# NVIDIA-Genomics-Research/DL4VC

Hardware: AMD Instinct MI355X
Metric: candidate-variants/sec (DAN fwd, 64 reads x 201 bp) (higher is better)
Workload: dtype f32

## Files before the change

### dl4vc_amd/capi.py

```python
from __future__ import annotations

import ctypes as C
import os
from typing import Dict, Optional

import numpy as np

from .config import DanConfig

_HERE = os.path.dirname(os.path.abspath(__file__))
LIB_PATH = os.path.join(_HERE, "csrc", "libdl4vc_dan.so")
ABI_VERSION = 6

SYMBOLS = ("dan_abi_version", "dan_source_hash", "dan_create", "dan_set_tensor", "dan_finalize", "dan_destroy", "dan_last_error",
           "dan_forward", "dan_forward_aux", "dan_forward_device", "dan_forward_async", "dan_wait", "dan_set_tap", "dan_read_buffer", "dan_query",
           "dan_profile_enable", "dan_kernel_stats")


class DanCConfig(C.Structure):
    _fields_ = [("reads", C.c_int32), ("length", C.c_int32), ("layers", C.c_int32), ("c_init", C.c_int32),
                ("c_final", C.c_int32), ("dil_mid", C.c_int32), ("dil_final", C.c_int32),
                ("pool_layers_mask", C.c_uint32), ("residual_start", C.c_int32), ("use_bn", C.c_int32),
                ("use_q", C.c_int32), ("use_strand", C.c_int32), ("use_mask", C.c_int32), ("bottleneck", C.c_int32),
                ("fc_sizes", C.c_int32 * 2), ("precision", C.c_int32), ("device_id", C.c_int32),
                ("max_batch", C.c_int32), ("chunk_sites", C.c_int32), ("conv_algo", C.c_int32), ("skip_empty_rows", C.c_int32),
                ("bf16_form", C.c_int32)]


_lib = None

# ... 16 lines not shown
    lib.dan_destroy.argtypes = [vp]
    lib.dan_destroy.restype = None
    lib.dan_last_error.argtypes = [vp]
    lib.dan_last_error.restype = C.c_char_p
    planes = [vp] * 6
    lib.dan_forward.argtypes = [vp] + planes + [C.c_int64] + [vp] * 4
    lib.dan_forward_aux.argtypes = [vp] + planes + [C.c_int64] + [vp] * 5
    lib.dan_forward_device.argtypes = [vp] + planes + [C.c_int64] + [vp] * 5 + [vp]
    lib.dan_forward_async.argtypes = [vp] + planes + [C.c_int64] + [vp] * 5 + [C.POINTER(C.c_int64)]
    lib.dan_wait.argtypes = [vp, C.c_int64]
    lib.dan_set_tap.argtypes = [vp, C.c_int32]
    lib.dan_read_buffer.argtypes = [vp, C.c_char_p, f32p, C.c_int64]
    lib.dan_read_buffer.restype = C.c_int64
    lib.dan_query.argtypes = [vp, C.c_char_p]
    lib.dan_query.restype = C.c_int64
    lib.dan_profile_enable.argtypes = [vp, C.c_int32]
    lib.dan_kernel_stats.argtypes = [vp, C.c_char_p, C.POINTER(C.c_int64), C.POINTER(C.c_double)]
    if lib.dan_abi_version() != ABI_VERSION:
        raise RuntimeError("libdl4vc_dan ABI %d != binding %d" % (lib.dan_abi_version(), ABI_VERSION))
    if path is None:
        _lib = lib
    return lib


def source_hash() -> str:
    return load_library().dan_source_hash().decode()


HASHED_SOURCES = ("dan_*.hip", "dan_*.h", "dan_capi.cpp", "dan_train_capi.cpp")

# ... 118 lines not shown
        ticket, out = token
        self._check(self.lib.dan_wait(self._h, ticket), "dan_wait")
        if "aux" in out:
            a = out.pop("aux")
            out.update(af=a[:, 0:1].copy(), cov=a[:, 1:2].copy(), vb=a[:, 2:12].copy(), vr=a[:, 12:22].copy())
        return out

    def forward_device(self, ptrs, n_sites: int, out_ptrs, stream: int = 0) -> None:
        v = lambda x: C.c_void_p(int(x)) if x else None
        rc = self.lib.dan_forward_device(self._h, *[v(x) for x in ptrs], int(n_sites), *[v(x) for x in out_ptrs], v(stream))
        self._check(rc, "dan_forward_device")

    def set_tap(self, layer: int) -> None:
        self._check(self.lib.dan_set_tap(self._h, layer), "dan_set_tap")

    def read_buffer(self, name: str, n_floats: int) -> np.ndarray:
        dst = np.empty(int(n_floats), np.float32)
        n = self.lib.dan_read_buffer(self._h, name.encode(), dst.ctypes.data_as(C.POINTER(C.c_float)), dst.size)
        if n < 0:
            self._check(int(n), "dan_read_buffer(%s)" % name)
        return dst[:n]

    def profile(self, on: bool) -> None:
        self._check(self.lib.dan_profile_enable(self._h, int(on)), "dan_profile_enable")

    def kernel_stats(self, kernel: str):
        n, ms = C.c_int64(0), C.c_double(0.0)
        self._check(self.lib.dan_kernel_stats(self._h, kernel.encode(), C.byref(n), C.byref(ms)), "dan_kernel_stats")
        return int(n.value), float(ms.value)
```

### dl4vc_amd/csrc/dan_capi.cpp

```cpp
#include "../../include/dl4vc_dan.h"
#include "dan_kernels.h"

#include <algorithm>
#include <cmath>
#include <cstdarg>
#include <cstdio>
#include <cstring>
#include <map>
#include <string>
#include <thread>
#include <vector>

using namespace dan;

namespace {

struct Tensor {
    std::vector<float> data;
    std::vector<int64_t> shape;
    int64_t numel() const { int64_t n = 1; for (auto s : shape) n *= s; return n; }
};

std::string g_create_error;

// ... 28 lines not shown
    char* d_wlr = nullptr;
    float* d_wc16 = nullptr;
    float *d_wpool = nullptr, *d_cols = nullptr, *d_cp = nullptr, *d_zero = nullptr;
    bool use_p = false;
    bool use_x = false;
    char* d_wlx = nullptr;
    unsigned res_mask = 0;
    float *d_emb = nullptr, *d_pe = nullptr;
    float* d_l0tab = nullptr;
    float *d_y = nullptr, *d_pool = nullptr, *d_h = nullptr, *d_tap = nullptr;
    float* d_y2 = nullptr;
    bool split = false;
    int* d_rowsrc = nullptr;
    int *d_work = nullptr, *d_work_count = nullptr;
    int n_cus = 0;
    float *d_wc = nullptr, *d_bc = nullptr;
    float *d_feat = nullptr, *d_hid0 = nullptr, *d_hid1 = nullptr;
    float* d_fc_ws = nullptr;
    float *d_w0 = nullptr, *d_b0 = nullptr, *d_w1 = nullptr, *d_b1 = nullptr, *d_wh = nullptr, *d_bh = nullptr;
    uint16_t* d_w0x = nullptr;
    uint8_t* d_in = nullptr;
    float* d_out = nullptr;
    struct Slot {
        uint8_t *pin_in = nullptr, *dev_in = nullptr;
        float *pin_out = nullptr, *dev_out = nullptr;
        hipEvent_t ev_h2d = nullptr, ev_comp = nullptr, ev_done = nullptr;
        std::vector<hipEvent_t> ev_slice;
        int64_t ticket = -1, n = 0;
        float* dst[5] = {nullptr, nullptr, nullptr, nullptr, nullptr};
    } slot[2];
// ... 220 lines not shown
    if ((c.pool_layers_mask & 1u) || (c.pool_layers_mask >> c.layers))
        return fail(nullptr, DAN_ERR_INVALID_ARG, "pool layers must lie in 1..layers-1");
    const bool wino_ok = c.precision == 0 && (c.layers < 3 || c.dil_mid == 2) && (c.layers < 2 || c.dil_final == 2);
    if (c.conv_algo < 0 || c.conv_algo > 2) return fail(nullptr, DAN_ERR_INVALID_ARG, "conv_algo %d unknown (0 = auto, 1 = direct, 2 = winograd)", c.conv_algo);
    if (c.skip_empty_rows < 0 || c.skip_empty_rows > 1) return fail(nullptr, DAN_ERR_INVALID_ARG, "skip_empty_rows must be 0 or 1");
    if (c.bf16_form < 0 || c.bf16_form > 1) return fail(nullptr, DAN_ERR_INVALID_ARG, "bf16_form %d unknown (0 = eight waves, 1 = sixteen waves)", c.bf16_form);
    if (c.bf16_form != 0 && c.precision != 2) return fail(nullptr, DAN_ERR_INVALID_ARG, "bf16_form selects a form of the precision-2 kernel");
    if (c.conv_algo == 2 && !wino_ok)
        return fail(nullptr, DAN_ERR_INVALID_ARG, "conv_algo 2 (winograd) needs precision 0 and dilation 2 on every conv layer after the first");
    int ndev = 0;
    if (hipGetDeviceCount(&ndev) != hipSuccess || ndev <= 0 || c.device_id < 0 || c.device_id >= ndev)
        return fail(nullptr, DAN_ERR_NO_DEVICE, "no HIP device %d (found %d): the DAN forward has no CPU path", c.device_id, ndev);
    dan_handle* h = new dan_handle();
    h->cfg = c;
    { int cus = 0; if (hipDeviceGetAttribute(&cus, hipDeviceAttributeMultiprocessorCount, c.device_id) == hipSuccess) h->n_cus = cus; }
    h->max_batch = c.max_batch > 0 ? c.max_batch : 4096;
    if (c.chunk_sites > 0) {
        h->chunk = c.chunk_sites;
    } else {
        const double elem = c.precision == 2 ? 2.0 : 4.0;
        const double y_copies = (c.precision != 2 && c.length > MPOS) ? 2.0 : 1.0;
        const double per_site = (double)c.reads * c.length * (y_copies * CPAD + (double)c.layers * (c.bottleneck > 0 ? HPAD : 0)) * elem;
        double budget = 48e9;
        size_t free_b = 0, total_b = 0;
        int prev_dev = -1;
        (void)hipGetDevice(&prev_dev);
        if (hipSetDevice(c.device_id) == hipSuccess && hipMemGetInfo(&free_b, &total_b) == hipSuccess && free_b > 0)
            budget = std::min(budget, (double)free_b / 3.0);
        if (prev_dev >= 0 && prev_dev != c.device_id) (void)hipSetDevice(prev_dev);
        h->chunk_auto = true;
// ... 280 lines not shown
                                                                 {"fcHidden2Coverage", 1}, {"fcHidden2VB", VOCAB}, {"fcHidden2VR", VOCAB}};
    std::vector<float> wh, bh;
    for (auto& hd : heads) {
        const Tensor* w = need(h, std::string(hd.name) + ".weight", {hd.n, n1}, &rc); if (!w) return rc;
        const Tensor* b = need(h, std::string(hd.name) + ".bias", {hd.n}, &rc); if (!b) return rc;
        wh.insert(wh.end(), w->data.begin(), w->data.end());
        bh.insert(bh.end(), b->data.begin(), b->data.end());
    }
    if ((rc = dev_upload(h, &h->d_wh, wh)) || (rc = dev_upload(h, &h->d_bh, bh))) return rc;

    const size_t read_floats = (size_t)L * CPAD;
    const size_t act_div = h->use_p ? 2 : 1;
    if ((rc = dev_alloc(h, &h->d_y, (size_t)h->chunk * R * read_floats / act_div))) return rc;
    if (h->split && (rc = dev_alloc(h, &h->d_y2, (size_t)h->chunk * R * read_floats))) return rc;
    if ((rc = dev_alloc(h, &h->d_pool, (size_t)h->chunk * read_floats))) return rc;
    if (conv_pool && h->n_segments > 1) {
        if ((rc = dev_alloc(h, &h->d_cp, (size_t)h->chunk * read_floats))) return rc;
        if ((rc = dev_alloc(h, &h->d_cols, (size_t)h->chunk * L * 3 * CPAD))) return rc;
    }
    if (c.skip_empty_rows) {
        float* tmp = nullptr;
        if ((rc = dev_alloc(h, &tmp, (size_t)h->chunk * R))) return rc;
        h->d_rowsrc = (int*)tmp;
        if ((rc = dev_alloc(h, &tmp, (size_t)h->chunk * R + 4))) return rc;
        h->d_work = (int*)tmp;
        h->d_work_count = h->d_work + (size_t)h->chunk * R;
    }
    if (H > 0 && (rc = dev_alloc(h, &h->d_h, (size_t)c.layers * h->chunk * R * L * HPAD / act_div))) return rc;
    if ((rc = dev_alloc(h, &h->d_feat, (size_t)h->max_batch * h->F_stride))) return rc;
    HIPCHK(h, hipMemset(h->d_feat, 0, (size_t)h->max_batch * h->F_stride * sizeof(float)));
// ... 13 lines not shown
    if (!h) return;
    (void)hipSetDevice(h->cfg.device_id);
    (void)hipDeviceSynchronize();
    for (void* p : h->allocs) (void)hipFree(p);
    if (h->async_ready) {
        for (auto& sl : h->slot) {
            (void)hipHostFree(sl.pin_in); (void)hipHostFree(sl.pin_out);
            (void)hipEventDestroy(sl.ev_h2d); (void)hipEventDestroy(sl.ev_comp); (void)hipEventDestroy(sl.ev_done);
            for (auto& e : sl.ev_slice) (void)hipEventDestroy(e);
        }
        (void)hipStreamDestroy(h->s_h2d); (void)hipStreamDestroy(h->s_comp); (void)hipStreamDestroy(h->s_d2h);
    }
    for (auto& kv : h->stats) for (auto& ev : kv.second.pending) { (void)hipEventDestroy(ev.a); (void)hipEventDestroy(ev.b); }
    for (auto& ev : h->event_pool) { (void)hipEventDestroy(ev.a); (void)hipEventDestroy(ev.b); }
    delete h;
}

struct ChunkFeed {
    int (*fn)(void* ctx, int64_t first_site, int n_sites, int64_t k, hipEvent_t* ready);
    void* ctx;
};
static int forward_device_impl(dan_t* h, const uint8_t* reads, const uint8_t* qual, const uint8_t* strand, const uint8_t* ref,
                               const uint8_t* ref_mask, const uint8_t* var_mask, int64_t n_sites, float* bin_logits,
                               float* vt_logits, float* vt_prob, float* bp, float* aux, void* stream, const ChunkFeed* feed);

int dan_forward_device(dan_t* h, const uint8_t* reads, const uint8_t* qual, const uint8_t* strand, const uint8_t* ref,
                       const uint8_t* ref_mask, const uint8_t* var_mask, int64_t n_sites, float* bin_logits,
                       float* vt_logits, float* vt_prob, float* bp, float* aux, void* stream) {
    return forward_device_impl(h, reads, qual, strand, ref, ref_mask, var_mask, n_sites, bin_logits, vt_logits, vt_prob, bp, aux, stream, nullptr);
}
// ... 16 lines not shown
        const int nb = (int)std::min<int64_t>(h->max_batch, n_sites - mb);
        for (int c0 = 0; c0 < nb; c0 += h->chunk) {
            const int ns = std::min(h->chunk, nb - c0);
            const int64_t g0 = mb + c0;
            if (feed) {
                hipEvent_t ready;
                int rcf = feed->fn(feed->ctx, g0, ns, g0 / h->chunk, &ready); if (rcf) return rcf;
                HIPCHK(h, hipStreamWaitEvent(s, ready, 0));
            }
            if (h->d_rowsrc) {
                EventPair evm{};
                int rcm = prof_begin(h, "row_map", s, &evm); if (rcm) return rcm;
                launch_row_map(reads + g0 * rl, qual + g0 * rl, strand + g0 * rl, h->d_rowsrc, h->d_work, h->d_work_count, ns, R, L, s);
                rcm = prof_end(h, "row_map", s, &evm); if (rcm) return rcm;
            }
            float* y_seg = h->d_y;
            for (int sg = 0; sg < h->n_segments; ++sg) {
                SegmentArgs a{};
                a.wl = h->d_wl;
                a.l_begin = h->seg_begin[sg]; a.l_end = h->seg_end[sg];
                a.n_layers = c.layers; a.dil_mid = c.dil_mid; a.dil_final = c.dil_final;
                a.res_mask = h->res_mask; a.has_hw = H > 0;
                a.R = R; a.L = L;
                a.reads = reads + g0 * rl; a.qual = qual + g0 * rl; a.strand = strand + g0 * rl;
                a.ref = ref + g0 * L; a.ref_mask = ref_mask + g0 * L; a.var_mask = var_mask + g0 * L;
                a.emb = h->d_emb; a.pe = h->d_pe;
                float* const y_in = y_seg;
                if (h->split) y_seg = (y_seg == h->d_y) ? h->d_y2 : h->d_y;
                a.y = y_in; a.y_out = y_seg;
                if (c.precision != 2 && !plan_units(a, L, segment_halo(c, a.l_begin, a.l_end)))
                    return fail(h, DAN_ERR_STATE, "unit plan failed for segment %d", sg);
                a.pool = sg > 0 ? h->d_pool : nullptr;
                a.h = h->d_h; a.h_layer_stride = h_layer_stride;
                const bool tap_here = h->tap_layer >= 0 &&
                                      ((h->tap_layer == 0 && sg == 0) || (h->tap_layer > a.l_begin && h->tap_layer <= a.l_end));
                a.tap = tap_here ? h->d_tap : nullptr;
                a.tap_layer = h->tap_layer;
                a.wino = h->wino;
                a.l0_tab = h->d_l0tab;
                a.work = h->d_work; a.work_count = h->d_rowsrc ? h->d_work_count : nullptr;
                EventPair ev{};
                int rc = prof_begin(h, "conv_segment", s, &ev); if (rc) return rc;
                if (c.precision == 0) {
                    launch_segment(a, ns, h->n_cus, s);
                } else if (h->use_x) {
                    SegmentXArgs b{};
                    b.wl = h->d_wlx; b.l_begin = a.l_begin; b.l_end = a.l_end; b.n_layers = a.n_layers;
                    b.dil_mid = a.dil_mid; b.dil_final = a.dil_final; b.res_mask = a.res_mask; b.has_hw = a.has_hw;
                    b.R = a.R; b.L = a.L; b.reads = a.reads; b.qual = a.qual; b.strand = a.strand; b.ref = a.ref;
                    b.ref_mask = a.ref_mask; b.var_mask = a.var_mask; b.emb = a.emb; b.pe = a.pe;
                    b.y = (uint16_t*)a.y; b.y_out = (uint16_t*)a.y_out; b.pool = sg > 0 ? h->d_cp : nullptr; b.h = h->d_h; b.h_layer_stride = a.h_layer_stride;
                    b.units = a.units; b.Lw = a.Lw;
                    for (int u = 0; u < 2; ++u) { b.u_off[u] = a.u_off[u]; b.u_len[u] = a.u_len[u]; b.own_lo[u] = a.own_lo[u]; b.own_hi[u] = a.own_hi[u]; }
                    b.tap = a.tap; b.tap_layer = a.tap_layer; b.work = a.work; b.work_count = a.work_count;
                    b.stagger = -1;
                    launch_segmentx(b, ns, h->n_cus, s);
                } else if (h->use_p) {
                    SegmentPArgs b{};
                    b.wl = h->d_wlp; b.wlr = h->d_wlr; b.form = c.bf16_form; b.l_begin = a.l_begin; b.l_end = a.l_end; b.n_layers = a.n_layers;
                    b.dil_mid = a.dil_mid; b.dil_final = a.dil_final; b.res_mask = a.res_mask; b.has_hw = a.has_hw;
                    b.R = a.R; b.L = a.L; b.reads = a.reads; b.qual = a.qual; b.strand = a.strand; b.ref = a.ref;
                    b.ref_mask = a.ref_mask; b.var_mask = a.var_mask; b.emb = a.emb; b.pe = a.pe;
                    b.y = (uint16_t*)h->d_y; b.pool = sg > 0 ? h->d_cp : nullptr; b.h = (uint16_t*)h->d_h; b.h_layer_stride = a.h_layer_stride;
                    b.tap = a.tap; b.tap_layer = a.tap_layer; b.work = a.work; b.work_count = a.work_count;
                    launch_segmentp(b, ns, h->n_cus, s);
                }
                rc = prof_end(h, "conv_segment", s, &ev); if (rc) return rc;
                if (sg + 1 < h->n_segments) {
                    rc = prof_begin(h, "pool", s, &ev); if (rc) return rc;
                    if (h->use_p || h->use_x) {
                        if (h->use_x) launch_read_meanx((const uint16_t*)y_seg, h->d_pool, ns, R, L, h->d_rowsrc, s);
                        else launch_read_mean16((const uint16_t*)h->d_y, h->d_pool, ns, R, L, h->d_rowsrc, s);
                        const int ln = h->seg_begin[sg + 1];
                        launch_conv_pool(h->d_pool, h->d_wpool + (size_t)(sg + 1) * CPAD * 3 * CPAD, h->d_zero, h->d_cols, h->d_cp, ns, L,
                                         ln + 1 < c.layers ? c.dil_mid : c.dil_final, s);
                    } else launch_read_mean(y_seg, h->d_pool, ns, R, L, h->d_rowsrc, s);
                    rc = prof_end(h, "pool", s, &ev); if (rc) return rc;
                    HIPCHK(h, hipGetLastError());
                }
            }
            float* feat = h->d_feat + (size_t)c0 * h->F_stride;
            EventPair ev{};
            int rc = prof_begin(h, "pool", s, &ev); if (rc) return rc;
            if (h->use_x) launch_final_poolx((const uint16_t*)y_seg, feat, h->F_stride, ns, R, L, c.c_final, h->d_rowsrc, s);
            else if (h->use_p) launch_final_pool16((const uint16_t*)h->d_y, feat, h->F_stride, ns, R, L, c.c_final, h->d_rowsrc, s);
            else launch_final_pool(y_seg, feat, h->F_stride, ns, R, L, c.c_final, h->d_rowsrc, s);
            rc = prof_end(h, "pool", s, &ev); if (rc) return rc;
            HIPCHK(h, hipGetLastError());
            if (H > 0) {
                rc = prof_begin(h, "highway", s, &ev); if (rc) return rc;
                if (h->use_p)
                    launch_highway16((const uint16_t*)h->d_h, h_layer_stride, h->d_wc16, (long long)L * 2 * 2 * 64 * 4, h->d_bc, feat,
                                     h->F_stride, 2 * c.c_final * L, ns, R, L, H, c.layers, h->d_rowsrc, s);
                else
                    launch_highway(h->d_h, h_layer_stride, h->d_wc, (long long)L * 2 * 2 * 64 * 4, h->d_bc, feat, h->F_stride,
                                   2 * c.c_final * L, ns, R, L, H, c.layers, h->d_rowsrc, s);
                rc = prof_end(h, "highway", s, &ev); if (rc) return rc;
            }
            h->last_chunk_sites = ns;
        }
        EventPair ev{};
        int rc = prof_begin(h, "fc", s, &ev); if (rc) return rc;
        if (h->d_w0x)
            launch_fcx(h->d_feat, h->F_stride, h->d_w0x, h->F_stride, (long long)c.fc_sizes[0] * h->F_stride, h->d_b0, h->d_hid0, h->n0_stride,
                       nb, c.fc_sizes[0], (int)h->F_stride, 1, s, h->d_fc_ws, (long long)2 * h->max_batch * c.fc_sizes[0]);
        else
            launch_fc(h->d_feat, h->F_stride, h->d_w0, h->F_stride, h->d_b0, h->d_hid0, h->n0_stride, nb, c.fc_sizes[0],
                      (int)h->F_stride, 1, s, h->d_fc_ws, (long long)2 * h->max_batch * c.fc_sizes[0]);
        launch_fc(h->d_hid0, h->n0_stride, h->d_w1, h->n0_stride, h->d_b1, h->d_hid1, c.fc_sizes[1], nb, c.fc_sizes[1],
                  h->n0_stride, 1, s);
        launch_heads(h->d_hid1, c.fc_sizes[1], h->d_wh, h->d_bh, nb, bin_logits ? bin_logits + mb * 2 : nullptr,
                     vt_logits ? vt_logits + mb * 3 : nullptr, vt_prob ? vt_prob + mb * 3 : nullptr,
                     bp ? bp + mb : nullptr, aux ? aux + mb * 22 : nullptr, s);
        rc = prof_end(h, "fc", s, &ev); if (rc) return rc;
// ... 175 lines not shown
}

int dan_set_tap(dan_t* h, int32_t layer) {
    if (!h) return DAN_ERR_INVALID_ARG;
    if (layer < -1 || layer > h->cfg.layers) return fail(h, DAN_ERR_INVALID_ARG, "tap layer %d out of range", layer);
    if (layer >= 0 && !h->d_tap) {
        if (!h->finalized) return fail(h, DAN_ERR_STATE, "dan_set_tap before dan_finalize");
        HIPCHK(h, hipSetDevice(h->cfg.device_id));
        int rc = dev_alloc(h, &h->d_tap, (size_t)h->chunk * h->cfg.reads * h->cfg.length * CPAD);
        if (rc) return rc;
    }
    h->tap_layer = layer;
    return DAN_OK;
}

int64_t dan_query(const dan_t* h, const char* what) {
    if (!h || !what) return DAN_ERR_INVALID_ARG;
    const std::string w(what);
    if (w == "feature_width") return h->F;
    if (w == "feature_stride") return h->F_stride;
    if (w == "chunk_sites") return h->chunk;
    if (w == "chunk_sites_auto") return h->chunk_auto ? 1 : 0;
    if (w == "max_batch") return h->max_batch;
    if (w == "cpad") return CPAD;
    if (w == "tap_sites") return h->last_chunk_sites;
    if (w == "segments") return h->n_segments;
    if (w == "bf16_pingpong") return h->use_p ? 1 : 0;
    if (w == "bf16x3_split_kernel") return h->use_x ? 1 : 0;
    if (w == "hidden0_stride") return h->n0_stride;
    return fail(h, DAN_ERR_INVALID_ARG, "dan_query: unknown key '%s'", what);
}

int64_t dan_read_buffer(dan_t* h, const char* name, float* dst, int64_t capacity) {
    if (!h || !name || !dst || capacity < 0) return DAN_ERR_INVALID_ARG;
    if (!h->finalized) return fail(h, DAN_ERR_STATE, "dan_read_buffer before dan_finalize");
    const dan_config& c = h->cfg;
    const std::string w(name);
    const float* src = nullptr;
    int64_t n = 0;
    if (w == "tap") { if (!h->d_tap) return fail(h, DAN_ERR_STATE, "no tap was requested"); src = h->d_tap; n = (int64_t)h->last_chunk_sites * c.reads * c.length * CPAD; }
    else if (w == "feature") { src = h->d_feat; n = h->last_batch * h->F_stride; }
    else if (w == "hidden0") { src = h->d_hid0; n = h->last_batch * h->n0_stride; }
    else if (w == "hidden1") { src = h->d_hid1; n = h->last_batch * c.fc_sizes[1]; }
    else if (w == "pool") { src = h->d_pool; n = (int64_t)h->last_chunk_sites * c.length * CPAD; }
// ... 54 lines not shown
```

### dl4vc_amd/csrc/dan_kernels.h

```cpp
#pragma once
#include <hip/hip_runtime.h>
#include <stdint.h>

namespace dan {

constexpr int CPAD = 128;
constexpr int NWAVE = 8;
constexpr int SEG_THREADS = NWAVE * 64;
constexpr int NT = 2;
constexpr int MTW = 7;
constexpr int MT = 13;
constexpr int MPOS = MT * 16;
constexpr int HALO = 4;
constexpr int LDS_S = 136;
constexpr int LDS_ROWS = MPOS + 2 * HALO;
constexpr int HPAD = 32;
constexpr int CIN0 = 48;
constexpr int KG0 = CIN0 / 16;
constexpr int KGC = CPAD / 16;
constexpr int EMBED = 20;
constexpr int VOCAB = 10;
constexpr int NHEAD = 27;

constexpr int W_OFF = 0;
// ... 20 lines not shown
    float* y;
    const float* pool;
    float* h;
    long long h_layer_stride;
    float* tap;
    int tap_layer;
    int wino;
    int n_rows;
    int xcd_rows;
    const int* work;
    const int* work_count;
    const float* l0_tab;
    int units, Lw;
    int u_off[2], u_len[2], own_lo[2], own_hi[2];
    float* y_out;
};

constexpr int L0_NTJ = 101;
constexpr int L0_TJ_OFF = 0;
constexpr int L0_WSC_OFF = L0_TJ_OFF + 3 * L0_NTJ * CPAD;
constexpr int L0_PE_OFF = L0_WSC_OFF + 5 * 3 * CPAD;
inline size_t l0_tab_floats(int Lw) { return (size_t)L0_PE_OFF + (size_t)3 * Lw * CPAD; }
constexpr int L0_TOK = 8;
constexpr int L0_MAX_LAYERS = (MAX_LAYERS * CST_FLOATS - (MPOS + 2) * L0_TOK) / CST_FLOATS;

template <class Args>
inline bool plan_units(Args& a, int Lw, int halo) {
    a.Lw = Lw;
    if (Lw <= MPOS) {
        a.units = 1; a.L = Lw;
        a.u_off[0] = 0; a.u_len[0] = Lw; a.own_lo[0] = 0; a.own_hi[0] = Lw;
        a.u_off[1] = 0; a.u_len[1] = 0; a.own_lo[1] = 0; a.own_hi[1] = 0;
        return true;
    }
    const int mid = (Lw + 1) / 2;
    const int len = mid + halo;
    if (len > MPOS || len > Lw) return false;
    a.units = 2; a.L = len;
    a.u_off[0] = 0; a.u_len[0] = len; a.own_lo[0] = 0; a.own_hi[0] = mid;
    a.u_off[1] = Lw - len; a.u_len[1] = len; a.own_lo[1] = mid - (Lw - len); a.own_hi[1] = len;
    return true;
}

void launch_segment(const SegmentArgs& a, int n_sites, int max_wgs, hipStream_t s);

constexpr int P_HALO = 4;
constexpr int P_ROW_BYTES = 256;
constexpr int P_LMAX = 304;
constexpr int P_ROWS = P_LMAX + 2 * P_HALO;
constexpr int P_IMG_BYTES = P_ROWS * P_ROW_BYTES;
constexpr int P_LDS_BYTES = 163840;
constexpr int P_KS0 = CIN0 / 16;
constexpr int P_KSC = CPAD / 16;
constexpr int WP_FRAG = 1024;
constexpr int WP_CONV_OFF = 0;
constexpr int WP_RES_OFF = WP_CONV_OFF + 3 * P_KSC * 4 * WP_FRAG;
constexpr int WP_BOT_OFF = WP_RES_OFF + P_KSC * 4 * WP_FRAG;
constexpr int WP_CST_OFF = WP_BOT_OFF + P_KSC * WP_FRAG;
constexpr int WP_LAYER_BYTES = WP_CST_OFF + (CST_FLOATS + 32) * 4;
// ... 95 lines not shown
```

### dl4vc_amd/csrc/dan_kernels.hip

```cpp
#include "dan_device.h"

namespace dan {

#ifdef DAN_STAMPS
__device__ unsigned long long* g_stamps;
constexpr int NSTAMP = 64;
#define STAMP(k)                                                                                      \
    do {                                                                                              \
        __builtin_amdgcn_sched_barrier(0);                                                            \
        unsigned long long t_ = __builtin_amdgcn_s_memtime();                                         \
        __builtin_amdgcn_s_waitcnt(0xC07F);                                                           \
        if (lane == 0 && (k) < NSTAMP) g_stamps[((size_t)stamp_row * NWAVE + wave) * NSTAMP + (k)] = t_; \
        __builtin_amdgcn_sched_barrier(0);                                                            \
    } while (0)
#else
#define STAMP(k) do {} while (0)
#endif

static_assert((HALO + WHB + 4 * (4 * MW - 1) + 1 + 4 + 1) * LDS_S <= LDS_ROWS * LDS_S + MAX_LAYERS * CST_FLOATS, "wino reads stay inside LDS");
static_assert(WHB + 4 * (4 * MW - 1) + 3 >= MPOS - 1 && 4 * (4 * MW - 1) + 3 >= WHB - 1, "wino tiling covers the read");
static_assert(WHB_SHORT + 4 * (4 * MW_SHORT - 1) + 3 >= MPOS_SHORT - 1 && 4 * (4 * MW_SHORT - 1) + 3 >= WHB_SHORT - 1 && WHB_SHORT % 4 == 2,
              "short wino tiling covers its unit");

template <int TW>
// ... 9 lines not shown
        a_nxt = wl[(size_t)gn * (KGC * 64)];
#pragma unroll
        for (int m = 0; m < TW; ++m) {
            __builtin_amdgcn_s_setprio(3);
#pragma unroll
            for (int s = 0; s < 4; ++s)
#pragma unroll
                for (int o = 0; o < 2; ++o) acc[m][o] = mfma16(a[s], b[m][o][s], acc[m][o]);
            __builtin_amdgcn_s_setprio(0);
#pragma unroll
            for (int o = 0; o < 2; ++o) b[m][o] = *(const v4f*)(xrow + (4 * m + 2 * o) * LDS_S + gn * 16);
        }
    }
}

template <bool WINO, bool PERSIST, bool SPLIT, int TW = MW>
__global__ __launch_bounds__(SEG_THREADS, NWAVE / 4) void segment_kernel(SegmentArgs a_by_value) {
    static_assert((!(SPLIT && WINO) && TW == MW) || (SPLIT && WINO && TW == MW_SHORT), "six tiles per lane: the split Winograd kernel, and only it");
    constexpr int TILES = TW == MW ? MT : (MPOS_SHORT + 15) / 16;
    __shared__ __attribute__((aligned(16))) float lds[LDS_ROWS * LDS_S + MAX_LAYERS * CST_FLOATS];
    float* const xs = lds;
    float* const cst = lds + LDS_ROWS * LDS_S;
    typedef const __attribute__((address_space(4))) SegmentArgs* kernarg_ptr;
    constexpr int UNITS = SPLIT ? 2 : 1;
    const int n_work = (a_by_value.work_count ? *a_by_value.work_count : a_by_value.n_rows) * UNITS;
    const int per = a_by_value.work_count ? (n_work + 7) >> 3 : a_by_value.xcd_rows * UNITS;
    const int xcd = blockIdx.x & 7;
    int j = blockIdx.x >> 3;
    int wk = xcd * per + j;
    if (j >= per || wk >= n_work) return;
next_row:
    {
    kernarg_ptr ap = (kernarg_ptr)__builtin_amdgcn_kernarg_segment_ptr();
    if (PERSIST) asm volatile("" : "+s"(ap));
    auto args = [&]() -> decltype(auto) { if constexpr (PERSIST) return (*ap); else return (a_by_value); };
    const auto& a = args();
    [[maybe_unused]] const int unit = wk & 1;
    const int L = SPLIT ? (unit ? a.u_len[1] : a.u_len[0]) : a.L;
    const int Lw = SPLIT ? a.Lw : L;
    const int u_off = SPLIT ? (unit ? a.u_off[1] : a.u_off[0]) : 0;
    [[maybe_unused]] const int own_lo = SPLIT ? (unit ? a.own_lo[1] : a.own_lo[0]) : 0;
    [[maybe_unused]] const int own_hi = SPLIT ? (unit ? a.own_hi[1] : a.own_hi[0]) : L;
    [[maybe_unused]] const int stamp_row = wk;
    int tid = threadIdx.x;
    if (PERSIST) asm volatile("" : "+v"(tid));
    const int lane = tid & 63;
    const int wave = __builtin_amdgcn_readfirstlane(tid >> 6);
    const int wrow = SPLIT ? wk >> 1 : wk;
    const int row_index = __builtin_amdgcn_readfirstlane(a.work_count ? a.work[wrow] : wrow);
    const int site = (int)((unsigned)row_index / (unsigned)a.R);
    const int r = row_index - site * a.R;
    const size_t read_idx = (size_t)site * a.R + r;
    float* yrow = a.y + (read_idx * (size_t)Lw + u_off) * CPAD;
    float* yout = SPLIT ? a.y_out + (read_idx * (size_t)Lw + u_off) * CPAD : yrow;
    const int pos = lane & 15, kk = lane >> 4;
    const int cq = wave & 3, ph = wave >> 2;
    const int m_base = ph * MTW, cnt = ph ? MT - MTW : MTW;
    int chb[NT];
#pragma unroll
    for (int n = 0; n < NT; ++n) chb[n] = (cq * NT + n) * 16 + kk * 4;

    STAMP(0);
    [[maybe_unused]] const int wP0 = wino_base<TW>(lane);
    [[maybe_unused]] const int wlim = ((lane >> 2) & 1) ? wino_cover(TW) : wino_half_base(TW);
    [[maybe_unused]] const int chw = wave * 16 + kk * 4;
    auto dil_of = [&](int l) { return (l == 0) ? 1 : (l + 1 < a.n_layers ? a.dil_mid : a.dil_final); };
// ... 117 lines not shown
    __syncthreads();
    STAMP(1);
    if (a.tap && a.tap_layer == 0 && a.l_begin == 0) copy_out(xs, a.tap + (read_idx * (size_t)Lw + u_off) * CPAD, own_lo, own_hi, tid);

    v4f wbot[KGC];
    auto layer_tail = [&](int l, const float* lc, bool late_prefetch) {
        [[maybe_unused]] const int sb = 2 + (l - a.l_begin) * 8;
        __syncthreads();
        STAMP(sb + 6);
        if (a.tap && a.tap_layer == l + 1) {
            int t = tid;
            asm volatile("" : "+v"(t));
            copy_out(xs, a.tap + (read_idx * (size_t)Lw + u_off) * CPAD, own_lo, own_hi, t);
        }
        if (WINO && CARRY && late_prefetch && l + 1 < a.l_end) first_frags(l + 1, pn0, pn1, pn2, pn3);
        if (a.has_hw && !(WINO && l + 1 < a.l_end))
            bottleneck<NWAVE, SPLIT, TILES>(xs, wbot, lc + CST_BBOT, a.h + (size_t)l * a.h_layer_stride + (read_idx * (size_t)Lw + u_off) * HPAD,
                                     own_hi, wave, lane, own_lo);
        STAMP(sb + 7);
        if (CARRY) { pc0 = pn0; pc1 = pn1; pc2 = pn2; pc3 = pn3; }
    };

    auto direct_layer = [&](int l) {
        const float* wblk = a.wl + (size_t)l * LAYER_STRIDE;
        const float* lc = cst + (l - a.l_begin) * CST_FLOATS;
        const bool residual = (a.res_mask >> l) & 1u;
        const int kg = (l == 0) ? KG0 : KGC;
        const int dil = dil_of(l);
        gv4f_ptr w_conv = (gv4f_ptr)(wblk + W_OFF) + (cq * NT) * 64 + lane;
        gv4f_ptr w_res = (gv4f_ptr)(wblk + WRES_OFF) + (cq * NT) * 64 + lane;
        gv4f_ptr w_bot = (gv4f_ptr)(wblk + WBOT_OFF) + lane;
// ... 292 lines not shown
            for (int g = 0; g < KGC; ++g) wbot[g] = w_bot[(g * 2 + (wave & 1)) * 64];
        }
        layer_tail(0, lc, true);
    };

    if constexpr (WINO) {
        int l = a.l_begin;
        if (l == 0) { if (l0_lookup) lookup_layer0(); else direct_layer(0); l = 1; }
        for (; l < a.l_end; ++l) wino_layer_body(l);
    } else {
        int l = a.l_begin;
        if (l == 0 && l0_lookup) { lookup_layer0(); l = 1; }
        for (; l < a.l_end; ++l) direct_layer(l);
    }
    STAMP(62);
    copy_out(xs, yout, own_lo, own_hi, tid);
    STAMP(63);
    }
    if constexpr (PERSIST) {
        j += gridDim.x >> 3;
        wk = xcd * per + j;
        __syncthreads();
        if (j < per && wk < n_work) goto next_row;
    }
}

void launch_segment(const SegmentArgs& a0, int n_sites, int max_wgs, hipStream_t s) {
    SegmentArgs a = a0;
    a.n_rows = n_sites * a.R;
    a.xcd_rows = ((n_sites + 7) / 8) * a.R;
    const bool split = a.units == 2;
    if (!split) { a.units = 1; a.Lw = a.L; a.y_out = a.y; }
    const int units = split ? 2 : 1;
    const bool persist = a.work_count != nullptr && max_wgs >= 8 && max_wgs < a.n_rows * units;
    const dim3 grid((unsigned)(persist ? (max_wgs & ~7) : 8 * a.xcd_rows * units)), blk(SEG_THREADS);
    if (split) {
        static_assert((304 + 1) / 2 + 1 + 2 * (MAX_LAYERS - 1) <= MPOS_SHORT, "a split Winograd unit fits the six-tile form");
        const bool wino = a.wino && a.L <= MPOS_SHORT;
        a.wino = wino;
        if (persist) {
            if (wino) hipLaunchKernelGGL((segment_kernel<true, true, true, MW_SHORT>), grid, blk, 0, s, a);
            else hipLaunchKernelGGL((segment_kernel<false, true, true>), grid, blk, 0, s, a);
        } else {
            if (wino) hipLaunchKernelGGL((segment_kernel<true, false, true, MW_SHORT>), grid, blk, 0, s, a);
            else hipLaunchKernelGGL((segment_kernel<false, false, true>), grid, blk, 0, s, a);
        }
    } else if (persist) {
        if (a.wino) hipLaunchKernelGGL((segment_kernel<true, true, false>), grid, blk, 0, s, a);
// ... 397 lines not shown
```

### include/dl4vc_dan.h

```cpp
#ifndef DL4VC_DAN_H
#define DL4VC_DAN_H

#include <stdint.h>

#ifdef __cplusplus
extern "C" {
#endif

#define DAN_ABI_VERSION 6
#define DAN_MAX_LAYERS 16

typedef enum dan_status {
    DAN_OK = 0,
    DAN_ERR_INVALID_ARG = -1,
    DAN_ERR_MISSING_TENSOR = -2,
    DAN_ERR_SHAPE = -3,
    DAN_ERR_STATE = -4,
    DAN_ERR_HIP = -5,
    DAN_ERR_NO_DEVICE = -6
} dan_status;

typedef struct dan_config {
    int32_t reads;
    int32_t length;
// ... 36 lines not shown
                    const uint8_t* ref, const uint8_t* ref_mask, const uint8_t* var_mask, int64_t n_sites,
                    float* bin_logits, float* vt_logits, float* vt_prob, float* bp, float* aux);
int dan_forward_device(dan_t* h, const uint8_t* reads, const uint8_t* qual, const uint8_t* strand,
                       const uint8_t* ref, const uint8_t* ref_mask, const uint8_t* var_mask,
                       int64_t n_sites, float* bin_logits, float* vt_logits, float* vt_prob, float* bp,
                       float* aux, void* stream);

int dan_forward_async(dan_t* h, const uint8_t* reads, const uint8_t* qual, const uint8_t* strand,
                      const uint8_t* ref, const uint8_t* ref_mask, const uint8_t* var_mask, int64_t n_sites,
                      float* bin_logits, float* vt_logits, float* vt_prob, float* bp, float* aux, int64_t* ticket);
int dan_wait(dan_t* h, int64_t ticket);

int dan_set_tap(dan_t* h, int32_t layer);
int64_t dan_read_buffer(dan_t* h, const char* name, float* dst, int64_t capacity);
int64_t dan_query(const dan_t* h, const char* what);

int dan_profile_enable(dan_t* h, int32_t on);
int dan_kernel_stats(dan_t* h, const char* kernel, int64_t* launches, double* total_ms);

#ifdef __cplusplus
}
#endif
#endif
```

Before: 13810.

## Fuse read pooling into the persistent conv segment kernel via site-owning workgroups

Adds a FOLD variant of the segment kernel in which each workgroup owns whole sites and processes their reads in sequence. It accumulates the per-site mean and max pooling in a per-workgroup scratch buffer, then writes pooled activations or final features directly. This removes the separate pool kernel launches and the round trip of full activations through memory. The cost is less parallelism: one workgroup serialises all R reads of a site, and the scratch is read and written once per read. An automatic heuristic enables it only when sites divide evenly across CUs.

```diff
diff --git a/dl4vc_amd/capi.py b/dl4vc_amd/capi.py
--- a/dl4vc_amd/capi.py
+++ b/dl4vc_amd/capi.py
@@ -14,6 +14,7 @@
 
 SYMBOLS = ("dan_abi_version", "dan_source_hash", "dan_create", "dan_set_tensor", "dan_finalize", "dan_destroy", "dan_last_error",
            "dan_forward", "dan_forward_aux", "dan_forward_device", "dan_forward_async", "dan_wait", "dan_set_tap", "dan_read_buffer", "dan_query",
+           "dan_set_pool_form",
            "dan_profile_enable", "dan_kernel_stats")
 
 
@@ -60,6 +61,8 @@
     lib.dan_read_buffer.restype = C.c_int64
     lib.dan_query.argtypes = [vp, C.c_char_p]
     lib.dan_query.restype = C.c_int64
+    if hasattr(lib, "dan_set_pool_form"):
+        lib.dan_set_pool_form.argtypes = [vp, C.c_int32]
     lib.dan_profile_enable.argtypes = [vp, C.c_int32]
     lib.dan_kernel_stats.argtypes = [vp, C.c_char_p, C.POINTER(C.c_int64), C.POINTER(C.c_double)]
     if lib.dan_abi_version() != ABI_VERSION:
@@ -208,6 +211,9 @@
     def set_tap(self, layer: int) -> None:
         self._check(self.lib.dan_set_tap(self._h, layer), "dan_set_tap")
 
+    def set_pool_form(self, form: int) -> None:
+        self._check(self.lib.dan_set_pool_form(self._h, form), "dan_set_pool_form")
+
     def read_buffer(self, name: str, n_floats: int) -> np.ndarray:
         dst = np.empty(int(n_floats), np.float32)
         n = self.lib.dan_read_buffer(self._h, name.encode(), dst.ctypes.data_as(C.POINTER(C.c_float)), dst.size)
diff --git a/dl4vc_amd/csrc/dan_capi.cpp b/dl4vc_amd/csrc/dan_capi.cpp
--- a/dl4vc_amd/csrc/dan_capi.cpp
+++ b/dl4vc_amd/csrc/dan_capi.cpp
@@ -66,6 +66,10 @@
     int* d_rowsrc = nullptr;
     int *d_work = nullptr, *d_work_count = nullptr;
     int n_cus = 0;
+    const char* fold_why_not = nullptr;
+    int pool_form = 0;
+    int last_pool_form = 1;
+    float* d_fold = nullptr;
     float *d_wc = nullptr, *d_bc = nullptr;
     float *d_feat = nullptr, *d_hid0 = nullptr, *d_hid1 = nullptr;
     float* d_fc_ws = nullptr;
@@ -316,6 +320,11 @@
     dan_handle* h = new dan_handle();
     h->cfg = c;
     { int cus = 0; if (hipDeviceGetAttribute(&cus, hipDeviceAttributeMultiprocessorCount, c.device_id) == hipSuccess) h->n_cus = cus; }
+    h->fold_why_not = c.precision != 0 ? "the in-segment pooling form exists for precision 0 only"
+                    : c.length > MPOS ? "the in-segment pooling form needs one unit per read (windows up to 208 columns)"
+                    : c.skip_empty_rows ? "the in-segment pooling form computes every row: not with skip_empty_rows"
+                    : h->n_cus < 8 ? "the in-segment pooling form needs at least 8 compute units" : nullptr;
+    h->last_pool_form = h->fold_why_not ? 1 : 2;
     h->max_batch = c.max_batch > 0 ? c.max_batch : 4096;
     if (c.chunk_sites > 0) {
         h->chunk = c.chunk_sites;
@@ -626,6 +635,7 @@
     if ((rc = dev_alloc(h, &h->d_y, (size_t)h->chunk * R * read_floats / act_div))) return rc;
     if (h->split && (rc = dev_alloc(h, &h->d_y2, (size_t)h->chunk * R * read_floats))) return rc;
     if ((rc = dev_alloc(h, &h->d_pool, (size_t)h->chunk * read_floats))) return rc;
+    if (!h->fold_why_not && (rc = dev_alloc(h, &h->d_fold, (size_t)(h->n_cus & ~7) * 2 * read_floats))) return rc;
     if (conv_pool && h->n_segments > 1) {
         if ((rc = dev_alloc(h, &h->d_cp, (size_t)h->chunk * read_floats))) return rc;
         if ((rc = dev_alloc(h, &h->d_cols, (size_t)h->chunk * L * 3 * CPAD))) return rc;
@@ -669,6 +679,14 @@
     for (auto& kv : h->stats) for (auto& ev : kv.second.pending) { (void)hipEventDestroy(ev.a); (void)hipEventDestroy(ev.b); }
     for (auto& ev : h->event_pool) { (void)hipEventDestroy(ev.a); (void)hipEventDestroy(ev.b); }
     delete h;
+}
+
+static constexpr double FOLD_GAIN = 0.013;
+static bool fold_deals_evenly(int ns, int n_cus) {
+    const int W = n_cus & ~7;
+    if (W < 8 || ns <= 0) return false;
+    const int per = (ns + 7) / 8, rounds = (per + W / 8 - 1) / (W / 8);
+    return (double)rounds * W / ns - 1.0 < FOLD_GAIN;
 }
 
 struct ChunkFeed {
@@ -715,6 +733,8 @@
                 launch_row_map(reads + g0 * rl, qual + g0 * rl, strand + g0 * rl, h->d_rowsrc, h->d_work, h->d_work_count, ns, R, L, s);
                 rcm = prof_end(h, "row_map", s, &evm); if (rcm) return rcm;
             }
+            const bool fold = !h->fold_why_not && (h->pool_form == 2 || (h->pool_form == 0 && fold_deals_evenly(ns, h->n_cus)));
+            float* const feat = h->d_feat + (size_t)c0 * h->F_stride;
             float* y_seg = h->d_y;
             for (int sg = 0; sg < h->n_segments; ++sg) {
                 SegmentArgs a{};
@@ -740,6 +760,11 @@
                 a.wino = h->wino;
                 a.l0_tab = h->d_l0tab;
                 a.work = h->d_work; a.work_count = h->d_rowsrc ? h->d_work_count : nullptr;
+                if (fold) {
+                    a.fold = 1; a.fold_scratch = h->d_fold;
+                    if (sg + 1 < h->n_segments) a.fold_pool = h->d_pool;
+                    else { a.fold_feat = feat; a.fold_feat_stride = h->F_stride; a.fold_C = c.c_final; }
+                }
                 EventPair ev{};
                 int rc = prof_begin(h, "conv_segment", s, &ev); if (rc) return rc;
                 if (c.precision == 0) {
@@ -767,7 +792,9 @@
                     launch_segmentp(b, ns, h->n_cus, s);
                 }
                 rc = prof_end(h, "conv_segment", s, &ev); if (rc) return rc;
-                if (sg + 1 < h->n_segments) {
+                if (fold) {
+                    HIPCHK(h, hipGetLastError());
+                } else if (sg + 1 < h->n_segments) {
                     rc = prof_begin(h, "pool", s, &ev); if (rc) return rc;
                     if (h->use_p || h->use_x) {
                         if (h->use_x) launch_read_meanx((const uint16_t*)y_seg, h->d_pool, ns, R, L, h->d_rowsrc, s);
@@ -780,14 +807,16 @@
                     HIPCHK(h, hipGetLastError());
                 }
             }
-            float* feat = h->d_feat + (size_t)c0 * h->F_stride;
             EventPair ev{};
-            int rc = prof_begin(h, "pool", s, &ev); if (rc) return rc;
-            if (h->use_x) launch_final_poolx((const uint16_t*)y_seg, feat, h->F_stride, ns, R, L, c.c_final, h->d_rowsrc, s);
-            else if (h->use_p) launch_final_pool16((const uint16_t*)h->d_y, feat, h->F_stride, ns, R, L, c.c_final, h->d_rowsrc, s);
-            else launch_final_pool(y_seg, feat, h->F_stride, ns, R, L, c.c_final, h->d_rowsrc, s);
-            rc = prof_end(h, "pool", s, &ev); if (rc) return rc;
-            HIPCHK(h, hipGetLastError());
+            int rc = DAN_OK;
+            if (!fold) {
+                rc = prof_begin(h, "pool", s, &ev); if (rc) return rc;
+                if (h->use_x) launch_final_poolx((const uint16_t*)y_seg, feat, h->F_stride, ns, R, L, c.c_final, h->d_rowsrc, s);
+                else if (h->use_p) launch_final_pool16((const uint16_t*)h->d_y, feat, h->F_stride, ns, R, L, c.c_final, h->d_rowsrc, s);
+                else launch_final_pool(y_seg, feat, h->F_stride, ns, R, L, c.c_final, h->d_rowsrc, s);
+                rc = prof_end(h, "pool", s, &ev); if (rc) return rc;
+                HIPCHK(h, hipGetLastError());
+            }
             if (H > 0) {
                 rc = prof_begin(h, "highway", s, &ev); if (rc) return rc;
                 if (h->use_p)
@@ -799,6 +828,7 @@
                 rc = prof_end(h, "highway", s, &ev); if (rc) return rc;
             }
             h->last_chunk_sites = ns;
+            h->last_pool_form = fold ? 2 : 1;
         }
         EventPair ev{};
         int rc = prof_begin(h, "fc", s, &ev); if (rc) return rc;
@@ -1004,6 +1034,15 @@
     return DAN_OK;
 }
 
+int dan_set_pool_form(dan_t* h, int32_t form) {
+    if (!h) return DAN_ERR_INVALID_ARG;
+    if (form < 0 || form > 2) return fail(h, DAN_ERR_INVALID_ARG, "pool form %d: 0 = automatic, 1 = separate kernels, 2 = in-segment", form);
+    if (form == 2 && h->fold_why_not) return fail(h, DAN_ERR_INVALID_ARG, "pool form 2 refused: %s", h->fold_why_not);
+    h->pool_form = form;
+    h->last_pool_form = (form == 1 || h->fold_why_not) ? 1 : 2;
+    return DAN_OK;
+}
+
 int64_t dan_query(const dan_t* h, const char* what) {
     if (!h || !what) return DAN_ERR_INVALID_ARG;
     const std::string w(what);
@@ -1018,6 +1057,7 @@
     if (w == "bf16_pingpong") return h->use_p ? 1 : 0;
     if (w == "bf16x3_split_kernel") return h->use_x ? 1 : 0;
     if (w == "hidden0_stride") return h->n0_stride;
+    if (w == "pool_form") return h->last_pool_form;
     return fail(h, DAN_ERR_INVALID_ARG, "dan_query: unknown key '%s'", what);
 }
 
diff --git a/dl4vc_amd/csrc/dan_kernels.h b/dl4vc_amd/csrc/dan_kernels.h
--- a/dl4vc_amd/csrc/dan_kernels.h
+++ b/dl4vc_amd/csrc/dan_kernels.h
@@ -58,6 +58,13 @@
     int units, Lw;
     int u_off[2], u_len[2], own_lo[2], own_hi[2];
     float* y_out;
+    int fold;
+    int n_sites, xcd_sites;
+    float* fold_scratch;
+    float* fold_pool;
+    float* fold_feat;
+    long long fold_feat_stride;
+    int fold_C;
 };
 
 constexpr int L0_NTJ = 101;
@@ -87,6 +94,7 @@
 }
 
 void launch_segment(const SegmentArgs& a, int n_sites, int max_wgs, hipStream_t s);
+int segment_fold_workgroups(int n_sites, int max_wgs);
 
 constexpr int P_HALO = 4;
 constexpr int P_ROW_BYTES = 256;
diff --git a/dl4vc_amd/csrc/dan_kernels.hip b/dl4vc_amd/csrc/dan_kernels.hip
--- a/dl4vc_amd/csrc/dan_kernels.hip
+++ b/dl4vc_amd/csrc/dan_kernels.hip
@@ -47,8 +47,9 @@
     }
 }
 
-template <bool WINO, bool PERSIST, bool SPLIT, int TW = MW>
+template <bool WINO, bool PERSIST, bool SPLIT, int TW = MW, bool FOLD = false>
 __global__ __launch_bounds__(SEG_THREADS, NWAVE / 4) void segment_kernel(SegmentArgs a_by_value) {
+    static_assert(!FOLD || (PERSIST && !SPLIT), "the site-owning form is a persistent one-unit form");
     static_assert((!(SPLIT && WINO) && TW == MW) || (SPLIT && WINO && TW == MW_SHORT), "six tiles per lane: the split Winograd kernel, and only it");
     constexpr int TILES = TW == MW ? MT : (MPOS_SHORT + 15) / 16;
     __shared__ __attribute__((aligned(16))) float lds[LDS_ROWS * LDS_S + MAX_LAYERS * CST_FLOATS];
@@ -56,12 +57,13 @@
     float* const cst = lds + LDS_ROWS * LDS_S;
     typedef const __attribute__((address_space(4))) SegmentArgs* kernarg_ptr;
     constexpr int UNITS = SPLIT ? 2 : 1;
-    const int n_work = (a_by_value.work_count ? *a_by_value.work_count : a_by_value.n_rows) * UNITS;
-    const int per = a_by_value.work_count ? (n_work + 7) >> 3 : a_by_value.xcd_rows * UNITS;
+    const int n_work = FOLD ? a_by_value.n_sites : (a_by_value.work_count ? *a_by_value.work_count : a_by_value.n_rows) * UNITS;
+    const int per = FOLD ? a_by_value.xcd_sites : a_by_value.work_count ? (n_work + 7) >> 3 : a_by_value.xcd_rows * UNITS;
     const int xcd = blockIdx.x & 7;
     int j = blockIdx.x >> 3;
     int wk = xcd * per + j;
     if (j >= per || wk >= n_work) return;
+    [[maybe_unused]] int fold_r = 0;
 next_row:
     {
     kernarg_ptr ap = (kernarg_ptr)__builtin_amdgcn_kernarg_segment_ptr();
@@ -80,9 +82,9 @@
     const int lane = tid & 63;
     const int wave = __builtin_amdgcn_readfirstlane(tid >> 6);
     const int wrow = SPLIT ? wk >> 1 : wk;
-    const int row_index = __builtin_amdgcn_readfirstlane(a.work_count ? a.work[wrow] : wrow);
-    const int site = (int)((unsigned)row_index / (unsigned)a.R);
-    const int r = row_index - site * a.R;
+    const int row_index = FOLD ? wk * a.R + fold_r : __builtin_amdgcn_readfirstlane(a.work_count ? a.work[wrow] : wrow);
+    const int site = FOLD ? wk : (int)((unsigned)row_index / (unsigned)a.R);
+    const int r = FOLD ? fold_r : row_index - site * a.R;
     const size_t read_idx = (size_t)site * a.R + r;
     float* yrow = a.y + (read_idx * (size_t)Lw + u_off) * CPAD;
     float* yout = SPLIT ? a.y_out + (read_idx * (size_t)Lw + u_off) * CPAD : yrow;
@@ -230,7 +232,7 @@
             copy_out(xs, a.tap + (read_idx * (size_t)Lw + u_off) * CPAD, own_lo, own_hi, t);
         }
         if (WINO && CARRY && late_prefetch && l + 1 < a.l_end) first_frags(l + 1, pn0, pn1, pn2, pn3);
-        if (a.has_hw && !(WINO && l + 1 < a.l_end))
+        if (!(FOLD && WINO) && a.has_hw && !(WINO && l + 1 < a.l_end) && !(FOLD && l + 1 == a.l_end))
             bottleneck<NWAVE, SPLIT, TILES>(xs, wbot, lc + CST_BBOT, a.h + (size_t)l * a.h_layer_stride + (read_idx * (size_t)Lw + u_off) * HPAD,
                                      own_hi, wave, lane, own_lo);
         STAMP(sb + 7);
@@ -553,15 +555,127 @@
         for (; l < a.l_end; ++l) direct_layer(l);
     }
     STAMP(62);
-    copy_out(xs, yout, own_lo, own_hi, tid);
+    if constexpr (FOLD) {
+        const bool fin = a.fold_feat != nullptr;
+        if (!fin) copy_out(xs, yout, own_lo, own_hi, tid);
+        constexpr int NF = MT * 16 * (CPAD / 4) / SEG_THREADS;
+        const int n4 = L * (CPAD / 4);
+        v4f* sp = (v4f*)(a.fold_scratch + (size_t)blockIdx.x * (2 * (size_t)n4 * 4));
+        int t = tid;
+        asm volatile("" : "+v"(t));
+        v4f fsum[NF], fmx[NF];
+        if (r > 0) {
+#pragma unroll
+            for (int k = 0; k < NF; ++k) {
+                const int i = t + k * SEG_THREADS;
+                fsum[k] = (i < n4) ? sp[i] : splat(0.f);
+            }
+        } else {
+#pragma unroll
+            for (int k = 0; k < NF; ++k) fsum[k] = splat(0.f);
+        }
+        if (r > 0 && fin) {
+#pragma unroll
+            for (int k = 0; k < NF; ++k) {
+                const int i = t + k * SEG_THREADS;
+                fmx[k] = (i < n4) ? sp[n4 + i] : splat(0.f);
+            }
+        } else {
+#pragma unroll
+            for (int k = 0; k < NF; ++k) fmx[k] = splat(0.f);
+        }
+        if (a.has_hw) {
+            const int ll = a.l_end - 1;
+            bottleneck<NWAVE, false, TILES>(xs, wbot, cst + (ll - a.l_begin) * CST_FLOATS + CST_BBOT,
+                                            a.h + (size_t)ll * a.h_layer_stride + read_idx * (size_t)Lw * HPAD, own_hi, wave, lane, own_lo);
+        }
+        const bool last_row = r + 1 == a.R;
+#pragma unroll
+        for (int k = 0; k < NF; ++k) {
+            const int i = t + k * SEG_THREADS;
+            const v4f v = (i < n4) ? *(const v4f*)(xs + (HALO + (i >> 5)) * LDS_S + (i & 31) * 4) : splat(0.f);
+            v4f mx = v;
+            if (r > 0) {
+#pragma unroll
+                for (int jj = 0; jj < 4; ++jj) mx[jj] = fmaxf(fmx[k][jj], v[jj]);
+            }
+            fmx[k] = mx;
+            v4f sum = fsum[k];
+            sum += v;
+            fsum[k] = (fin && r == 0) ? v : sum;
+        }
+        if (!last_row) {
+#pragma unroll
+            for (int k = 0; k < NF; ++k) {
+                const int i = t + k * SEG_THREADS;
+                if (i < n4) sp[i] = fsum[k];
+            }
+            if (fin) {
+#pragma unroll
+                for (int k = 0; k < NF; ++k) {
+                    const int i = t + k * SEG_THREADS;
+                    if (i < n4) sp[n4 + i] = fmx[k];
+                }
+            }
+        } else {
+            const float fR = (float)a.R;
+            __syncthreads();
+            auto put = [&](const v4f (&src)[NF]) {
+#pragma unroll
+                for (int k = 0; k < NF; ++k) {
+                    const int i = t + k * SEG_THREADS;
+                    if (i < n4) *(v4f*)(xs + (HALO + (i >> 5)) * LDS_S + (i & 31) * 4) = src[k];
+                }
+            };
+            if (!fin) {
+                put(fsum);
+                v4f* pl = (v4f*)(a.fold_pool + (size_t)site * n4 * 4);
+#pragma unroll 1
+                for (int i = t; i < n4; i += SEG_THREADS)
+                    pl[i] = *(const v4f*)(xs + (HALO + (i >> 5)) * LDS_S + (i & 31) * 4) / splat(fR);
+            } else {
+                float* row = a.fold_feat + (size_t)site * a.fold_feat_stride;
+                const int C = a.fold_C;
+                put(fmx);
+                __syncthreads();
+#pragma unroll 1
+                for (int c = wave; c < C; c += NWAVE)
+#pragma unroll 1
+                    for (int p = lane; p < L; p += 64) row[(unsigned)(c * L + p)] = xs[(HALO + p) * LDS_S + c];
+                __syncthreads();
+                put(fsum);
+                __syncthreads();
+                row += (size_t)C * L;
+#pragma unroll 1
+                for (int c = wave; c < C; c += NWAVE)
+#pragma unroll 1
+                    for (int p = lane; p < L; p += 64) row[(unsigned)(c * L + p)] = xs[(HALO + p) * LDS_S + c] / fR;
+            }
+        }
+    } else {
+        copy_out(xs, yout, own_lo, own_hi, tid);
+    }
     STAMP(63);
     }
-    if constexpr (PERSIST) {
+    if constexpr (FOLD) {
+        if (++fold_r == a_by_value.R) {
+            fold_r = 0;
+            j += gridDim.x >> 3;
+            wk = xcd * per + j;
+        }
+        __syncthreads();
+        if (j < per && wk < n_work) goto next_row;
+    } else if constexpr (PERSIST) {
         j += gridDim.x >> 3;
         wk = xcd * per + j;
         __syncthreads();
         if (j < per && wk < n_work) goto next_row;
     }
+}
+
+int segment_fold_workgroups(int n_sites, int max_wgs) {
+    const int w = max_wgs & ~7, need = 8 * ((n_sites + 7) / 8);
+    return w < need ? w : need;
 }
 
 void launch_segment(const SegmentArgs& a0, int n_sites, int max_wgs, hipStream_t s) {
@@ -571,6 +685,14 @@
     const bool split = a.units == 2;
     if (!split) { a.units = 1; a.Lw = a.L; a.y_out = a.y; }
     const int units = split ? 2 : 1;
+    if (a.fold) {
+        a.n_sites = n_sites;
+        a.xcd_sites = (n_sites + 7) / 8;
+        const dim3 grid((unsigned)segment_fold_workgroups(n_sites, max_wgs)), blk(SEG_THREADS);
+        if (a.wino) hipLaunchKernelGGL((segment_kernel<true, true, false, MW, true>), grid, blk, 0, s, a);
+        else hipLaunchKernelGGL((segment_kernel<false, true, false, MW, true>), grid, blk, 0, s, a);
+        return;
+    }
     const bool persist = a.work_count != nullptr && max_wgs >= 8 && max_wgs < a.n_rows * units;
     const dim3 grid((unsigned)(persist ? (max_wgs & ~7) : 8 * a.xcd_rows * units)), blk(SEG_THREADS);
     if (split) {
diff --git a/include/dl4vc_dan.h b/include/dl4vc_dan.h
--- a/include/dl4vc_dan.h
+++ b/include/dl4vc_dan.h
@@ -74,6 +74,7 @@
 int dan_set_tap(dan_t* h, int32_t layer);
 int64_t dan_read_buffer(dan_t* h, const char* name, float* dst, int64_t capacity);
 int64_t dan_query(const dan_t* h, const char* what);
+int dan_set_pool_form(dan_t* h, int32_t form);
 
 int dan_profile_enable(dan_t* h, int32_t on);
 int dan_kernel_stats(dan_t* h, const char* kernel, int64_t* launches, double* total_ms);
```

Result: faster. 14070 (median of 6 runs) (+1.9%).
